# keonlee9420/Comprehensive-Transformer-TTS

Measured on AMD Instinct MI355X. Metric: mel-frames/sec (train step) LJSpeech batch=16, 1/2/4/8 MI355X, higher is better.
Workload: dtype f32; 1 GPU; LJSpeech transformer_fs2 batch=16/GPU seq<=128->mel<=1024x80; full train step fwd+loss+bwd+clip+Adam, dropout on; workload_detail=supervised durations (BASELINE configs[1]), global_batch=16, valid_frames_per_gpu=11992, padded_frames_per_gpu=16384, launch_mode=hipgraph(fwd+bwd | clip+adam), parallelism=dp1

## Files before the change

comprehensive-transformer-tts_amd/_lib.py:

```python
import ctypes as C
import os

_HERE = os.path.dirname(os.path.abspath(__file__))
LIB_PATH = os.environ.get("CTTS_LIB") or os.path.join(_HERE, "csrc", "libctts_hip.so")

_c_f32p = C.c_void_p
_i32, _i64, _f32, _u32, _vp = C.c_int32, C.c_int64, C.c_float, C.c_uint32, C.c_void_p


class GemmDesc(C.Structure):
    _fields_ = [
        ("A", _vp), ("B", _vp), ("C", _vp),
        ("M", _i32), ("N", _i32), ("K", _i32),
        ("lda", _i64), ("ldb", _i64), ("ldc", _i64),
        ("a_kc", _i32), ("b_kc", _i32),
        ("nb0", _i32), ("nb1", _i32),
        ("sA0", _i64), ("sA1", _i64), ("sB0", _i64), ("sB1", _i64), ("sC0", _i64), ("sC1", _i64),
        ("lens", _vp),
        ("lim_m", _i32), ("lim_n", _i32), ("lim_k", _i32),
        ("conv_T", _i32), ("conv_pad", _i32), ("conv_cin", _i32), ("conv_on_b", _i32),
        ("split_k", _i32),
        ("alpha", _f32),
        ("bias", _vp),
        ("Z", _vp), ("ldz", _i64),
# ... 83 lines not shown
    "ctts_gemm_takes_weight_stationary": [C.POINTER(GemmDesc)],
    "ctts_gemm_takes_bf16_split": [C.POINTER(GemmDesc)],
    "ctts_gemm_takes_planes": [C.POINTER(GemmDesc)],
    "ctts_split_planes": [C.POINTER(SplitTask), C.c_int, _vp],
    "ctts_rowdot_heads": [_vp, _vp, _vp, C.c_int, C.c_int, C.c_int, C.c_int, _vp],
    "ctts_mel_prepare": [_vp, C.c_int, C.c_int, _vp, _vp],
    "ctts_mel_spectrogram": [_vp, _vp, _vp, _vp, _vp, _vp, _vp, _i64, C.c_int, C.c_int, C.c_int, C.c_int, C.c_int, _f32, C.c_int, _vp, _vp],
    "ctts_mha_fwd": [_vp, _vp, _vp, _vp, C.c_int, C.c_int, C.c_int, C.c_int, _f32, _vp],
    "ctts_mha_bwd": [_vp, _vp, _vp, _vp, _vp, _vp, _vp, _vp, _vp, C.c_int, C.c_int, C.c_int, C.c_int, _f32, C.c_int, _vp, _vp],
    "ctts_relmha_fwd": [_vp, _vp, _vp, _vp, _vp, _vp, C.c_int, C.c_int, C.c_int, C.c_int, _f32, _f32, _vp, _u32, _vp],
    "ctts_relmha_bwd": [_vp, _vp, _vp, _vp, _vp, _vp, _vp, _vp, _vp, _vp, _vp, _vp, _vp, C.c_int, C.c_int, C.c_int, C.c_int,
                        _f32, _f32, _vp, _u32, _vp],
    "ctts_weighted_colsum": [_vp, _vp, _vp, _i64, C.c_int, _f32, C.c_int, _vp, _vp, _vp],
    "ctts_epilogue_bwd": [_vp, _vp, _vp, _vp, _vp, _vp, _i64, C.c_int, C.c_int, _f32, _vp, _u32, _f32, C.c_int, _vp, _vp, _vp],
    "ctts_row_tile_map": [_vp, C.c_int, C.c_int, C.c_int, _vp, _vp],
    "ctts_batch_tile_map": [_vp] + [C.c_int] * 9 + [_vp, C.c_size_t, _vp],
    "ctts_conv_weight_repack": [_vp, _vp, C.c_int, C.c_int, C.c_int, C.c_int, _vp],
    "ctts_lr_index": [_vp, C.c_int, C.c_int, _vp, C.c_int, C.c_int, C.c_int, _vp, _vp, _vp, _vp],
    "ctts_lr_gather_fwd": [_vp, _vp, _vp, C.c_int, C.c_int, C.c_int, C.c_int, _vp],
    "ctts_lr_gather_bwd": [_vp, _vp, _vp, C.c_int, C.c_int, C.c_int, C.c_int, _vp],
    "ctts_embedding_fwd": [_vp, _vp, _vp, _i64, C.c_int, C.c_int, _vp],
    "ctts_embedding_bwd": [_vp, _vp, _vp, _i64, C.c_int, C.c_int, C.c_int, C.c_int, _vp, _vp],
    "ctts_positions": [_vp, C.c_int, _i64, C.c_int, C.c_int, _vp, _vp],
    "ctts_cwt_pitch": [_vp, _i64, C.c_int, _vp, _vp, _f32, _vp, C.c_int, _f32, _f32, _f32, C.c_int, _vp, _vp, _vp, C.c_int, C.c_int, C.c_int, _vp],
    "ctts_layernorm_fwd": [_vp, _vp, _vp, _vp, _vp, _vp, C.c_int, C.c_int, _f32, _f32, _vp, _u32, _vp, _vp, _vp],
    "ctts_layernorm_bwd": [_vp, _vp, _vp, _vp, _vp, _vp, _vp, _vp, C.c_int, C.c_int, _f32, _vp, _u32, _vp, C.c_int, _vp, _vp, _vp, _vp],
    "ctts_colstats": [_vp, _vp, C.c_int, C.c_int, _vp, _vp],
    "ctts_bn_finalize": [_vp, C.c_int, C.c_int, _f32, _f32, _vp, _vp, _vp, _vp, _vp, _vp],
    "ctts_bn_apply": [_vp, _vp, _vp, _vp, _vp, _vp, C.c_int, C.c_int, C.c_int, _f32, _vp, _u32, _vp, _vp],
    "ctts_bn_bwd_reduce": [_vp, _vp, _vp, _vp, _vp, _vp, _vp, C.c_int, C.c_int, C.c_int, _f32, _vp, _u32, _vp, _vp],
    "ctts_bn_bwd_apply": [_vp, _vp, _vp, _vp, _vp, _vp, _vp, _vp, _vp, _vp, C.c_int, C.c_int, C.c_int, _f32, _vp,
# ... 140 lines not shown
    lib.ctts_pitch_track_workspace_bytes.restype = C.c_size_t
    lib.ctts_pitch_track_workspace_bytes.argtypes = []
    lib.ctts_trim_silence_workspace_bytes.restype = C.c_size_t
    lib.ctts_trim_silence_workspace_bytes.argtypes = [C.c_int, C.c_int, C.c_int]
    lib.ctts_dtw_workspace_bytes.restype = C.c_size_t
    lib.ctts_dtw_workspace_bytes.argtypes = [C.c_int, C.c_int, C.c_int]
    lib.ctts_loudness_workspace_bytes.restype = C.c_size_t
    lib.ctts_loudness_workspace_bytes.argtypes = [C.c_int, C.c_int]
    lib.ctts_stoi_workspace_bytes.restype = C.c_size_t
    lib.ctts_stoi_workspace_bytes.argtypes = [C.c_int, C.c_int]
    lib.ctts_si_sdr_workspace_bytes.restype = C.c_size_t
    lib.ctts_si_sdr_workspace_bytes.argtypes = [C.c_int, C.c_int]
    lib.ctts_mr_stft_workspace_bytes.restype = C.c_size_t
    lib.ctts_mr_stft_workspace_bytes.argtypes = [C.c_int, C.c_int, C.c_int, C.c_int]
    lib.ctts_batch_tile_map_ints.restype = C.c_size_t
    lib.ctts_batch_tile_map_ints.argtypes = [C.c_int, C.c_int, C.c_int, C.c_int]
    lib.ctts_relmha_workspace_floats.restype = C.c_size_t
    lib.ctts_relmha_workspace_floats.argtypes = [C.c_int, C.c_int, C.c_int]
    _lib = lib
    return lib


def check(status, what):
    if status != 0:
        msg = load().ctts_last_error().decode(errors="replace")
        raise CttsError(f"{what} failed with status {status}: {msg}")
```

comprehensive-transformer-tts_amd/csrc/batch_plan.h:

```cpp
#pragma once
#include <stdint.h>
#ifdef __HIPCC__
#define BP_HD __host__ __device__ __forceinline__
#else
#define BP_HD inline
#endif

struct BatchPlanGeom {
  int M, N, K;
  int BM, BN, BK;
  int nbatch, nb1;
  int lim_m, lim_n, lim_k;
  int write_all;
  int nbins;
};

constexpr int BATCH_PLAN_HDR = 4;

BP_HD int batch_plan_tiles_m(const BatchPlanGeom& g) { return (g.M + g.BM - 1) / g.BM; }
BP_HD int batch_plan_tiles_n(const BatchPlanGeom& g) { return (g.N + g.BN - 1) / g.BN; }
BP_HD long batch_plan_items(const BatchPlanGeom& g) { return (long)g.nbatch * batch_plan_tiles_m(g) * batch_plan_tiles_n(g); }

BP_HD bool batch_plan_fits(const BatchPlanGeom& g) {
  const long tiles = (long)batch_plan_tiles_m(g) * batch_plan_tiles_n(g);
// ... 36 lines not shown
  for (int y = 0; y < g.nbatch; ++y) {
    const BatchPlanBatch o = batch_plan_batch(g, lens[y / g.nb1]);
    const int a = o.act_m * o.act_n;
    total += a;
    if (o.work > me.work || (o.work == me.work && y < z)) act_before += a;
    if (y < z) rest_before += tiles - a;
  }
  n_active = total;
  const int tm = tile / tiles_n, tn = tile - tm * tiles_n;
  const int act_in = (tm < me.act_m ? tm : me.act_m) * me.act_n + (tm < me.act_m ? (tn < me.act_n ? tn : me.act_n) : 0);
  if (tm < me.act_m && tn < me.act_n) return batch_plan_snake(act_before + act_in, total, g.nbins);
  return total + rest_before + (tile - act_in);
}

BP_HD int batch_plan_listed(const BatchPlanGeom& g, int n_active) { return g.write_all ? (int)batch_plan_items(g) : n_active; }
```

comprehensive-transformer-tts_amd/csrc/gemm.hip:

```cpp
#include "ctts_common.h"
#include "gemm_common.h"
#include "batch_plan.h"
#include <stdlib.h>
#include <type_traits>

namespace {

#ifndef CTTS_BK
#define CTTS_BK 32
#endif
#ifndef CTTS_GEMM_WAVES
#define CTTS_GEMM_WAVES 2
#endif
constexpr int BK = CTTS_BK;
constexpr int KC_LD = BK + 4;
constexpr int KCH = BK / 4;
static_assert(BK == 32 || BK == 64, "BK must be 32 or 64");


__device__ __forceinline__ bool rows_in_padding(const int32_t* row_lens, int row_T, int row_halo, int first, int last) {
  const int b0 = first / row_T;
  return b0 == last / row_T && (first - b0 * row_T) >= row_lens[b0] + row_halo;
}

// ... 379 lines not shown
__device__ __forceinline__ void fetch_frag(const float* s, int ext0, int l31, int h, int ksub, float (&f)[16]) {
  if (KC) {
    const float4* p = reinterpret_cast<const float4*>(s + (ext0 + l31) * LD + ksub + h * 16);
#pragma unroll
    for (int q = 0; q < 4; ++q) {
      float4 v = p[q];
      f[4 * q + 0] = v.x; f[4 * q + 1] = v.y; f[4 * q + 2] = v.z; f[4 * q + 3] = v.w;
    }
  } else {
    const float* p = s + (ksub + h * 16) * LD + ext0 + l31;
#pragma unroll
    for (int j = 0; j < 16; ++j) f[j] = p[j * LD];
  }
}

template <int BM, int BN, bool A_KC, bool B_KC, bool CONV, Fetch FETCH>
__global__ __launch_bounds__(256, CTTS_GEMM_WAVES) void gemm_tile_kernel(const ctts_gemm_desc d) {
  using FT = FetchTraits<FETCH>;
  constexpr int WAVES_N = BN >= 64 ? 2 : 1, WAVES_M = 4 / WAVES_N;
  constexpr int WM = BM / WAVES_M, WN = BN / WAVES_N, MT = WM / 32, NT = WN / 32;
  constexpr int A_LD = A_KC ? KC_LD : BM + 4;
  constexpr int B_LD = B_KC ? KC_LD : BN + 4;
  constexpr int A_SZ = A_KC ? BM * KC_LD : BK * (BM + 4);
  constexpr int B_SZ = B_KC ? BN * KC_LD : BK * (BN + 4);
  __shared__ __attribute__((aligned(16))) float smem[A_SZ + B_SZ];
  float* sA = smem;
  float* sB = smem + A_SZ;
  int z = blockIdx.z;
  const int split = blockIdx.y;
  const bool limited = FT::kLensLimits && (FT::kLensGiven || d.lens);
  const int tiles_n = (d.N + BN - 1) / BN;
  int wg, tm;
  bool scheduled_active = false;
  if constexpr (FT::kNaturalOrder) {
    wg = blockIdx.x;
    if (d.tile_map && !natural_order(d)) {
      const int32_t* plan = d.tile_map;
      const unsigned lin = blockIdx.z * gridDim.x + blockIdx.x;
      if (plan[2] == (int32_t)(gridDim.x * gridDim.z) && plan[3] == batch_plan_key(batch_plan_geom(d, BM, BN, 1))) {
        if (lin >= (unsigned)plan[1]) return;
        batch_plan_unpack(plan[BATCH_PLAN_HDR + lin], z, wg);
        if (z >= (int)gridDim.z || wg >= (int)gridDim.x) return;
      }
    }
    tm = wg / tiles_n;
// ... 2 lines not shown
    int r = wg / tiles_n;
    if (d.tile_group_n > 0) {
      const int g = d.tile_group_n, ngroups = tiles_n / g, mways = 8 / ngroups;
      const int x = blockIdx.x & 7, i = blockIdx.x >> 3;
      r = (i / g) * mways + x / ngroups;
      wg = r * tiles_n + (x % ngroups) * g + i % g;
    }
    tm = d.tile_map[1 + r];
    scheduled_active = FT::kTrustSchedule && r < d.tile_map[0];
  } else if (FT::kTileOrders && natural_order(d)) {
    wg = blockIdx.x;
    tm = wg / tiles_n;
  } else {
    xcd_tile_order(gridDim.x, tiles_n, true, wg, tm);
  }
  const int z0 = z / d.nb1, z1 = z - z0 * d.nb1;
  int Mv, Nv, Kv;
  batch_limits(d, z0, limited, Mv, Nv, Kv);
  const int row0 = tm * BM, col0 = (wg % tiles_n) * BN;
  float* Cb = d.C + z0 * d.sC0 + z1 * d.sC1;
  const bool zero_outside = limited && d.split_overwrite && d.split_k <= 1;
  if (row0 >= Mv || col0 >= Nv) {
    if (zero_outside && row0 < d.M && col0 < d.N) zero_outside_limits(d, Cb, row0, col0, BM, BN, Mv, Nv, true);
    return;
  }
  if (zero_outside && (row0 + BM > Mv || col0 + BN > Nv)) zero_outside_limits(d, Cb, row0, col0, BM, BN, Mv, Nv, false);
  float* Cs = Cb;
  if (d.split_k > 1) Cs += (long)split * d.M * d.ldc;
  if (A_KC && d.row_lens && !scheduled_active &&
      padded_tile_zeroed(d, FT::kPadFillOwnSplit ? Cs : Cb, row0, col0, BM, min(BN, Nv - col0), Mv)) return;
  int k_begin, k_end;
  if (!split_k_range(d, Kv, BK, split, k_begin, k_end)) return;

  ConvView cv{d.conv_T, d.conv_pad, d.conv_cin};
  ConvView nocv{1, 0, 1};
  constexpr bool CONV_A = CONV && A_KC;
  constexpr bool CONV_B = CONV && !A_KC && !B_KC;
  using LA = Loader<FETCH, A_KC, BM, CONV_A>;
  using LB = Loader<FETCH, B_KC, BN, CONV_B>;
  LA la; LB lb;
  la.init(d.A + z0 * d.sA0 + z1 * d.sA1, d.lda, row0, Mv, CONV_A ? cv : nocv, threadIdx.x);
  lb.init(d.B + z0 * d.sB0 + z1 * d.sB1, d.ldb, col0, Nv, CONV_B ? cv : nocv, threadIdx.x);

  const int lane = threadIdx.x & 63, wave = threadIdx.x >> 6;
  const int l31 = lane & 31, h = lane >> 5;
  const int wm0 = (wave / WAVES_N) * WM, wn0 = (wave % WAVES_N) * WN;
  floatx16 acc[MT][NT];
#pragma unroll
  for (int i = 0; i < MT; ++i)
#pragma unroll
    for (int j = 0; j < NT; ++j)
#pragma unroll
      for (int r = 0; r < 16; ++r) acc[i][j][r] = 0.f;

  constexpr bool KSKIP = !A_KC && !B_KC;
  auto kblock_active = [&](int k0) -> bool {
    if (!KSKIP || !d.row_lens) return true;
    return !rows_in_padding(d.row_lens, d.row_T, d.row_halo, k0, min(k0 + BK, k_end) - 1);
  };
  float4 ra[LA::NV], rb[LB::NV];
  bool act_cur = kblock_active(k_begin);
  if (act_cur) {
    la.load(k_begin, k_end, ra);
    lb.load(k_begin, k_end, rb);
    la.store(sA, ra);
    lb.store(sB, rb);
  }
  __syncthreads();
  for (int k0 = k_begin; k0 < k_end; k0 += BK) {
    const bool has_next = (k0 + BK) < k_end;
    const bool act_next = has_next && kblock_active(k0 + BK);
    if (act_next) {
      la.load(k0 + BK, k_end, ra);
      lb.load(k0 + BK, k_end, rb);
    }
    if (act_cur) {
#pragma unroll
      for (int ksub = 0; ksub < BK; ksub += 32) {
        float fa[MT][16], fb[NT][16];
#pragma unroll
        for (int i = 0; i < MT; ++i) fetch_frag<A_KC, A_LD>(sA, wm0 + i * 32, l31, h, ksub, fa[i]);
#pragma unroll
        for (int j = 0; j < NT; ++j) fetch_frag<B_KC, B_LD>(sB, wn0 + j * 32, l31, h, ksub, fb[j]);
#ifdef CTTS_GEMM_SETPRIO
        __builtin_amdgcn_s_setprio(CTTS_GEMM_SETPRIO);
#endif
#pragma unroll
        for (int kk = 0; kk < 16; ++kk)
#pragma unroll
          for (int i = 0; i < MT; ++i)
#pragma unroll
            for (int j = 0; j < NT; ++j)
              acc[i][j] = __builtin_amdgcn_mfma_f32_32x32x2f32(fa[i][kk], fb[j][kk], acc[i][j], 0, 0, 0);
#ifdef CTTS_GEMM_SETPRIO
        __builtin_amdgcn_s_setprio(0);
#endif
      }
    }
    if (KSKIP && !act_cur && !act_next) continue;
    __syncthreads();
    if (act_next) {
      la.store(sA, ra);
      lb.store(sB, rb);
    }
    __syncthreads();
    act_cur = act_next;
  }
  gemm_epilogue_auto<MT, NT>(d, acc, Cs, z, row0, col0, wm0, wn0, l31, h, Mv, Nv);
}

constexpr int X6_PROW = 64, X6_PLANE = 128 * X6_PROW;
__device__ __forceinline__ int x6_chunk(int row, int c) { return c ^ ((row >> 2) & 3); }
typedef __bf16 x6_bf16x8 __attribute__((ext_vector_type(8)));

typedef __bf16 x6_bf16x2 __attribute__((ext_vector_type(2)));
typedef float x6_floatx2 __attribute__((ext_vector_type(2)));
__device__ __forceinline__ unsigned x6_round_pair(float& a, float& b) {
  const x6_floatx2 v = {a, b};
  const unsigned p = __builtin_bit_cast(unsigned, __builtin_convertvector(v, x6_bf16x2));
  a -= __uint_as_float(p << 16);
  b -= __uint_as_float(p & 0xFFFF0000u);
  return p;
}
// ... 370 lines not shown
    const unsigned long long m = __ballot(a);
    if (a) map[1 + n_act + __popcll(m & ((1ULL << lane) - 1ULL))] = tm;
    n_act += __popcll(m);
  }
  int n_in = 0;
  for (int base = 0; base < tiles; base += 64) {
    const int tm = base + lane;
    const bool a = tm < tiles && inactive(tm);
    const unsigned long long m = __ballot(a);
    if (a) map[1 + n_act + n_in + __popcll(m & ((1ULL << lane) - 1ULL))] = tm;
    n_in += __popcll(m);
  }
  if (lane == 0) map[0] = n_act;
}

__global__ __launch_bounds__(256) void batch_tile_map_kernel(const BatchPlanGeom g, const int32_t* __restrict__ lens, int32_t* __restrict__ map) {
  const int n_items = (int)batch_plan_items(g), tiles = n_items / g.nbatch;
  for (int i = blockIdx.x * 256 + threadIdx.x; i < n_items; i += gridDim.x * 256) {
    const int z = i / tiles, tile = i - z * tiles;
    int n_active;
    const int slot = batch_plan_slot(g, lens, z, tile, n_active);
    map[BATCH_PLAN_HDR + slot] = batch_plan_pack(z, tile);
    if (i == 0) {
      map[0] = n_active;
      map[1] = batch_plan_listed(g, n_active);
      map[2] = n_items;
      map[3] = batch_plan_key(g);
    }
  }
}

__global__ __launch_bounds__(256) void splitk_reduce_kernel(const ctts_gemm_desc d, int BM, int kround) {
  const int z = blockIdx.z, z0 = z / d.nb1, z1 = z - z0 * d.nb1;
  int Mv, Nv, Kv;
  batch_limits(d, z0, true, Mv, Nv, Kv);
  const bool ow = d.split_overwrite != 0;
  const int nact = Kv > 0 ? gemm_split_range(Kv, d.split_k, kround, 0).nonempty : 0;
  if (nact == 0 && !ow) return;
  const long ldp = gemm_partial_ld(d.N);
  const int n4 = (int)(ldp >> 2);
// ... 49 lines not shown
}

static BatchPlanGeom batch_map_geom(int nb0, int nb1, int M, int N, int K, int lim_m, int lim_n, int lim_k, int write_all) {
  static int cus = 0;
  if (!cus) {
    int dev = 0;
    hipDeviceProp_t prop;
    cus = (hipGetDevice(&dev) == hipSuccess && hipGetDeviceProperties(&prop, dev) == hipSuccess && prop.multiProcessorCount > 0)
              ? prop.multiProcessorCount : 256;
    cus = ctts_env_int("CTTS_BATCH_BINS", cus);
    if (cus < 1) cus = 256;
  }
  return BatchPlanGeom{M, N, K, 64, 64, BK, nb0 * nb1, nb1, lim_m != 0, lim_n != 0, lim_k != 0, write_all != 0, cus};
}

extern "C" size_t ctts_batch_tile_map_ints(int nb0, int nb1, int M, int N) {
  if (nb0 < 1 || nb1 < 1 || M < 1 || N < 1 || (long)nb0 * nb1 > 32767) return 0;
  const BatchPlanGeom g = batch_map_geom(nb0, nb1, M, N, 1, 0, 0, 0, 0);
  return batch_plan_fits(g) ? (size_t)(BATCH_PLAN_HDR + batch_plan_items(g)) : 0;
}

extern "C" int ctts_batch_tile_map(const int32_t* lens, int nb0, int nb1, int M, int N, int K, int lim_m, int lim_n, int lim_k,
                                   int write_all, int32_t* tile_map, size_t map_ints, void* stream) {
  CTTS_REQUIRE(lens && tile_map && K >= 0, "ctts_batch_tile_map: bad arguments");
  const size_t need = ctts_batch_tile_map_ints(nb0, nb1, M, N);
  CTTS_REQUIRE(need > 0, "ctts_batch_tile_map: %d x %d batches of [%d, %d] do not fit a plan (ctts_batch_tile_map_ints)", nb0, nb1, M, N);
  CTTS_REQUIRE(map_ints >= need, "ctts_batch_tile_map: tile_map holds %zu int32, %zu needed", map_ints, need);
  const BatchPlanGeom g = batch_map_geom(nb0, nb1, M, N, K, lim_m, lim_n, lim_k, write_all);
  const long blocks = (batch_plan_items(g) + 255) / 256;
  hipLaunchKernelGGL(batch_tile_map_kernel, dim3((unsigned)(blocks < 64 ? blocks : 64)), dim3(256), 0, (hipStream_t)stream, g, lens, tile_map);
  CTTS_CHECK_LAUNCH("ctts_batch_tile_map");
  return 0;
}

static bool x6_plan(const ctts_gemm_desc& d) {
  const int on = d.bf16_split;
  static const long min_tiles = ctts_env_int("CTTS_X6_MIN_TILES", 384);
  if (on < 1 || !d.a_kc || !d.b_kc || d.nb0 * d.nb1 != 1 || d.split_k > 1 || d.E || d.lens || d.conv_on_b) return false;
  if (d.K < 256 || d.K % BK || d.N % 128 || d.M < 1024) return false;
  if (d.conv_T > 0 && d.conv_cin % 4) return false;
  if (on != 2 && on != 4 && (long)((d.M + 127) / 128) * (d.N / 128) < min_tiles) return false;
  return vec_ok(d) && buf_ok(d);
}

static bool x6tn_plan(const ctts_gemm_desc& d) {
// ... 164 lines not shown
    case CTTS_GEMM_SCALAR64: rc = for_layout<true>(t, [&](auto a, auto b, auto c) { return launch_tile<64, 64, a(), b(), c(), Fetch::Scalar>(t, st); }); break;
#ifndef CTTS_NO_BUF
    case CTTS_GEMM_BUF128: rc = for_layout<true>(t, [&](auto a, auto b, auto c) { return launch_tile<128, 128, a(), b(), c(), Fetch::Buffer>(t, st); }); break;
    case CTTS_GEMM_BUF_K2: rc = for_layout<true>(t, [&](auto a, auto b, auto c) { return launch_buf_k2<a(), b(), c()>(t, st); }); break;
    case CTTS_GEMM_BUF_NARROW: rc = for_layout<false>(t, [&](auto a, auto b, auto c) { return launch_tile<128, 32, a(), b(), c(), Fetch::Buffer>(t, st); }); break;
    case CTTS_GEMM_BUF64: rc = for_layout<true>(t, [&](auto a, auto b, auto c) { return launch_tile<64, 64, a(), b(), c(), Fetch::Buffer>(t, st); }); break;
#endif
    case CTTS_GEMM_VEC128: rc = for_layout<true>(t, [&](auto a, auto b, auto c) { return launch_tile<128, 128, a(), b(), c(), Fetch::Vec>(t, st); }); break;
    case CTTS_GEMM_X6TN: rc = x6tn_launch(t, st); break;
    default: rc = for_layout<true>(t, [&](auto a, auto b, auto c) { return launch_tile<64, 64, a(), b(), c(), Fetch::Vec>(t, st); }); break;
  }
  if (rc != 0 || !split || d.split_out) return rc;
  return splitk_reduce(d_user, r.info.tile_m, r.info.k_granule, st);
}

extern "C" int ctts_gemm_route(const ctts_gemm_desc* dp, ctts_gemm_route_info* info) {
  CTTS_REQUIRE(info != nullptr, "ctts_gemm_route: null info");
  *info = ctts_gemm_route_info{CTTS_GEMM_NONE, 0, 0, 0, 0};
  ctts_gemm_desc d;
  GemmRoute r;
  const int rc = gemm_plan(dp, d, r);
  if (rc == 0) *info = r.info;
  return rc < 0 ? rc : 0;
}

static int route_kind(const ctts_gemm_desc* dp) {
  if (!dp) return CTTS_GEMM_NONE;
  const ctts_gemm_desc d = gemm_normalized(*dp);
  GemmRoute r;
  gemm_route(d, r);
// ... 25 lines not shown
```

comprehensive-transformer-tts_amd/kernels.py:

```python
import collections
import ctypes as C

import torch

from . import _lib
from ._lib import GemmDesc

ACT_NONE, ACT_RELU, ACT_GELU, ACT_TANH, ACT_SWISH = 0, 1, 2, 3, 4


def _stream():
    return C.c_void_p(torch.cuda.current_stream().cuda_stream)


def _p(t, offset=0):
    if t is None:
        return None
    if not t.is_cuda:
        raise _lib.CttsError("ctts kernels need device (HIP) tensors; got a CPU tensor - no CPU fallback exists")
    return t.data_ptr() + offset * t.element_size()


def _f32c(t, name):
    if t.dtype != torch.float32 or not t.is_contiguous():
# ... 391 lines not shown
def gemm_takes_weight_stationary(A, B, Cout, M, N, K, lda, ldb, ldc, a_kc=True, b_kc=True, **kw):
    return _gemm_takes("weight_stationary", (A, B, Cout, M, N, K, lda, ldb, ldc, a_kc, b_kc), kw)


def gemm_ws_enable(on):
    return bool(_lib.load().ctts_gemm_ws_enable(1 if on else 0))


def row_tile_map(row_lens, row_T, row_halo, M):
    tm = torch.empty(1 + (M + 63) // 64, dtype=torch.int32, device=row_lens.device)
    lib = _lib.load()
    _lib.check(lib.ctts_row_tile_map(_p(row_lens), int(row_T), int(row_halo), int(M), _p(tm), _stream()), "ctts_row_tile_map")
    return tm


def batch_tile_map(lens, nb1, M, N, K, lim, write_all):
    lib = _lib.load()
    n = lib.ctts_batch_tile_map_ints(int(lens.numel()), int(nb1), int(M), int(N))
    if n == 0:
        return None
    tm = torch.empty(n, dtype=torch.int32, device=lens.device)
    _lib.check(lib.ctts_batch_tile_map(_p(lens), int(lens.numel()), int(nb1), int(M), int(N), int(K), int(lim[0]), int(lim[1]), int(lim[2]),
                                       int(bool(write_all)), _p(tm), n, _stream()), "ctts_batch_tile_map")
    return tm


def conv_dgrad_weights(weights):
    if not weights:
        return []
    outs = [torch.empty(cin, k * cout, dtype=torch.float32, device=w.device) for w, cout, cin, k in weights]
    arr = (_lib.RepackTask * len(weights))()
    for t, (w, cout, cin, k), o in zip(arr, weights, outs):
        t.src, t.dst, t.cout, t.cin, t.k = _p(_f32c(w, "conv weight (GEMM-major)")), _p(o), int(cout), int(cin), int(k)
    _lib.check(_lib.load().ctts_conv_dgrad_weights(arr, len(arr), _stream()), "ctts_conv_dgrad_weights")
    return outs


def conv_weight_repack(src, dst, cout, cin, k, mode):
    lib = _lib.load()
# ... 1481 lines not shown
```

comprehensive-transformer-tts_amd/ops.py:

```python
import contextlib
import math
import os as _os

import torch

from . import kernels as K
from .kernels import ACT_NONE, ACT_RELU, ACT_GELU, ACT_TANH, ACT_SWISH


_FUSE_GRAD_ACCUM = False


def set_grad_accumulation_fusion(flag):
    global _FUSE_GRAD_ACCUM
    _FUSE_GRAD_ACCUM = bool(flag)


def grad_accumulation_fusion():
    return _FUSE_GRAD_ACCUM


def _grad_of(p):
    if not _FUSE_GRAD_ACCUM or p is None or not p.requires_grad:
        return None
# ... 448 lines not shown
        _PLANES[kind][w.data_ptr()] = (pl, _wstamp(w))


def clear_dgrad_weights():
    _DGRAD_W.clear()
    _PLANES["fwd"].clear()
    _PLANES["dgrad"].clear()


class PadRows:

    def __init__(self, lens, T):
        self.lens, self.T = lens, int(T)
        self._maps = {}
        self._batch_maps = {}

    def tile_map(self, halo, M):
        key = (int(halo), int(M))
        if key not in self._maps:
            self._maps[key] = K.row_tile_map(self.lens, self.T, halo, M)
        return self._maps[key]


    def batch_map(self, A, B, Cout, lim, write_all):
        key = (tuple(Cout.shape), int(A.shape[-1]), tuple(lim), bool(write_all))
        if key not in self._batch_maps:
            plan = None
            nb1, (M, N), Kd = (Cout.shape[1] if Cout.dim() == 4 else 1), Cout.shape[-2:], A.shape[-1]
            if Cout.is_cuda and Cout.dim() >= 3 and Cout.shape[0] * nb1 * -(-M // 64) * -(-N // 64) > _BATCH_ORDER_MIN_ITEMS:
                args, views = K.gemm_views(A, B, Cout, lens=self.lens)
                route = K.gemm_route(*args, **views, lens=self.lens, lim=lim, split_overwrite=write_all)
                if route.kind == "buf64":
                    plan = K.batch_tile_map(self.lens, nb1, M, N, Kd, lim, write_all)
            self._batch_maps[key] = plan
        return self._batch_maps[key]


def _pad_rows(pad_rows):
    if pad_rows is None or isinstance(pad_rows, PadRows):
        return pad_rows
    return PadRows(pad_rows[0], pad_rows[1])


def linear(x, w, b=None, act=ACT_NONE, alpha=1.0, residual=None, rowscale=None, p_drop=0.0, drop=None, pad_rows=None, link=None,
           link_role=0):
    p_drop, seed, off = _drop_args(p_drop, drop)
    return _LinearConv.apply(x, w, b, residual, rowscale, act, alpha, p_drop, seed, off, 0, 0, _pad_rows(pad_rows), link, link_role)


def conv1d(x, w, b=None, act=ACT_NONE, alpha=1.0, residual=None, rowscale=None, p_drop=0.0, drop=None, pad_rows=None, link=None,
# ... 109 lines not shown


def layer_norm_res(x, gamma, beta, eps, planes_for=None):
    want = planes_for is not None and consumer_takes_planes(x, *planes_for)
    return _LayerNormRes.apply(x, gamma, beta, eps, want)


def layer_norm(x, gamma, beta, eps, rowscale=None, p_drop=0.0, drop=None):
    p_drop, seed, off = _drop_args(p_drop, drop)
    return _LayerNorm.apply(x, gamma, beta, eps, rowscale, p_drop, seed, off)


_ATTN_SPLIT_K = int(_os.environ.get("CTTS_ATTN_SPLIT_K", "1"))
_BATCH_ORDER = _os.environ.get("CTTS_BATCH_ORDER", "balanced")
_BATCH_ORDER_MIN_ITEMS = 256


def _attn_split_k(nbatch, T, dh):
    tiles = -(-T // 64) * -(-dh // 64) * nbatch
    return _ATTN_SPLIT_K if (_ATTN_SPLIT_K > 1 and tiles < 1536 and T >= 512) else 1


_FUSED_ATTN = {"1": True, "0": False}.get(_os.environ.get("CTTS_FUSED_ATTN", "auto"), None)
_ATTN_Q_SPLIT = int(_os.environ.get("CTTS_ATTN_Q_SPLIT", "0"))


def set_fused_attention(flag):
    global _FUSED_ATTN
    _FUSED_ATTN = flag if flag is None else bool(flag)

# ... 49 lines not shown
        ctx.n_heads = n_heads
        ctx.pad_rows = pr
        return out

    @staticmethod
    def backward(ctx, dO):
        qkv, P, lens, O = ctx.saved_tensors
        H, pr, bg = ctx.n_heads, ctx.pad_rows, _SelfAttention._bgemm
        dO = dO.contiguous()
        B, T, C3 = qkv.shape
        dh = C3 // 3 // H
        scale = dh ** -0.5
        sk = _attn_split_k(B * H, T, dh)
        dqkv = torch.empty_like(qkv)
        (q, k, v), (dq, dk, dv), (dOh,) = _heads(qkv, H, 3), _heads(dqkv, H, 3), _heads(dO, H)
        bg(pr, P.transpose(-1, -2), dOh, dv, lens, (1, 0, 1), split_k=sk, split_overwrite=True)
        Dv = K.rowdot_heads(dO, O, H)
        dP = torch.empty_like(P)
        bg(pr, dOh, v.transpose(-1, -2), dP, lens, (1, 1, 0), E=P, rowsub=Dv)
        bg(pr, dP, k, dq, lens, (1, 0, 1), alpha=scale, split_k=sk, split_overwrite=True)
        bg(pr, dP.transpose(-1, -2), q, dk, lens, (1, 0, 1), alpha=scale, split_k=sk, split_overwrite=True)
        return dqkv, None, None, None


def self_attention(qkv, lens_i32, n_heads, pad_rows=None):
    want = _FUSED_ATTN if _FUSED_ATTN is not None else not (torch.is_grad_enabled() and qkv.requires_grad)
    if want and K.mha_supported(qkv.shape[-1] // 3, n_heads):
        return _FusedSelfAttention.apply(qkv, lens_i32, n_heads)
    return _SelfAttention.apply(qkv, lens_i32, n_heads, pad_rows)


class _LRGather(torch.autograd.Function):
    @staticmethod
    def forward(ctx, x, mel2ph, cum):
# ... 829 lines not shown
```

include/ctts.h:

```cpp
#ifndef CTTS_H
#define CTTS_H
#include <stddef.h>
#include <stdint.h>

#ifdef __cplusplus
extern "C" {
#endif

const char* ctts_last_error(void);
int ctts_version(void);

typedef struct ctts_gemm_desc {
  const float* A; const float* B; float* C;
  int32_t M, N, K;
  int64_t lda, ldb, ldc;
  int32_t a_kc, b_kc;
  int32_t nb0, nb1;
  int64_t sA0, sA1, sB0, sB1, sC0, sC1;
  const int32_t* lens;
  int32_t lim_m, lim_n, lim_k;
  int32_t conv_T, conv_pad, conv_cin, conv_on_b;
  int32_t split_k;
  float alpha;
  const float* bias;
// ... 49 lines not shown
int ctts_gemm_takes_planes(const ctts_gemm_desc* d);
typedef struct ctts_split_task { const float* src; uint16_t* dst; int64_t rows, cols, ld; } ctts_split_task;
int ctts_split_planes(const ctts_split_task* tasks, int ntasks, void* stream);

int ctts_rowdot_heads(const float* a, const float* b, float* out, int B, int T, int H, int dh, void* stream);

int ctts_weighted_colsum(const float* x, const float* w, float* out, int64_t rows, int C, float scale, int accumulate, void* ws, float* parts,
                         void* stream);

int ctts_epilogue_bwd(const float* dy, const float* rowscale, const float* z, float* dz, float* gm, float* dbias, int64_t rows, int C,
                      int act, float p_drop, const uint64_t* seed, uint32_t drop_offset, float bias_scale, int accumulate_bias,
                      void* ws, float* parts, void* stream);

int ctts_row_tile_map(const int32_t* row_lens, int row_T, int row_halo, int M, int32_t* tile_map, void* stream);

size_t ctts_batch_tile_map_ints(int nb0, int nb1, int M, int N);
int ctts_batch_tile_map(const int32_t* lens, int nb0, int nb1, int M, int N, int K, int lim_m, int lim_n, int lim_k, int write_all,
                        int32_t* tile_map, size_t map_ints, void* stream);

int ctts_conv_weight_repack(const float* src, float* dst, int cout, int cin, int k, int mode, void* stream);

int ctts_lr_index(const void* dur, int dur_is_float, int round_mode, const uint8_t* pad, int B, int Ts, int Tm,
                  int32_t* mel2ph, int64_t* mel_len, int32_t* cum, void* stream);
int ctts_lr_gather_fwd(const float* x, const int32_t* mel2ph, float* out, int B, int Ts, int Tm, int C, void* stream);
int ctts_lr_gather_bwd(const float* dy, const int32_t* cum, float* dx, int B, int Ts, int Tm, int C, void* stream);

int ctts_cwt_pitch(const float* spec, int64_t ld_spec, int nscale, const float* f0_mean, const float* f0_std, float std_scale,
                   const float* uv, int uv_chan, float eps, float mel_min, float mel_max, int f0_bin, float* f0, float* f0_denorm,
                   int64_t* ids, int B, int T, int width, void* stream);

int ctts_positions(const void* src, int src_is_float, int64_t stride, int B, int T, int32_t* pos, void* stream);

int ctts_layernorm_fwd(const float* x, const float* gamma, const float* beta, float* y, float* mean, float* rstd,
// ... 247 lines not shown
```

Baseline: 672,200 mel-frames/s.

## Group attention-backward dV, dQ, dK batched GEMMs into one length-balanced launch

Adds a grouped GEMM kernel that runs up to three same-shape, length-limited batched GEMMs in one launch, using a combined tile plan that orders active tiles by work across all groups. Attention backward uses it for dV, dQ and dK, deferring dV until after dP is computed, when split-K is off. The aim is to cut launch count and fill the GPU better with small per-head attention GEMMs. In exchange the kernel is launched with bounds of 8 waves per SIMD and carries larger shared memory covering both layouts, and the tile-map API gains a groups argument.

```diff
diff --git a/comprehensive-transformer-tts_amd/_lib.py b/comprehensive-transformer-tts_amd/_lib.py
--- a/comprehensive-transformer-tts_amd/_lib.py
+++ b/comprehensive-transformer-tts_amd/_lib.py
@@ -121,7 +121,8 @@
     "ctts_weighted_colsum": [_vp, _vp, _vp, _i64, C.c_int, _f32, C.c_int, _vp, _vp, _vp],
     "ctts_epilogue_bwd": [_vp, _vp, _vp, _vp, _vp, _vp, _i64, C.c_int, C.c_int, _f32, _vp, _u32, _f32, C.c_int, _vp, _vp, _vp],
     "ctts_row_tile_map": [_vp, C.c_int, C.c_int, C.c_int, _vp, _vp],
-    "ctts_batch_tile_map": [_vp] + [C.c_int] * 9 + [_vp, C.c_size_t, _vp],
+    "ctts_batch_tile_map": [_vp] + [C.c_int] * 10 + [_vp, C.c_size_t, _vp],
+    "ctts_gemm_grouped": [_vp, C.c_int, _vp, _vp],
     "ctts_conv_weight_repack": [_vp, _vp, C.c_int, C.c_int, C.c_int, C.c_int, _vp],
     "ctts_lr_index": [_vp, C.c_int, C.c_int, _vp, C.c_int, C.c_int, C.c_int, _vp, _vp, _vp, _vp],
     "ctts_lr_gather_fwd": [_vp, _vp, _vp, C.c_int, C.c_int, C.c_int, C.c_int, _vp],
@@ -292,7 +293,7 @@
     lib.ctts_mr_stft_workspace_bytes.restype = C.c_size_t
     lib.ctts_mr_stft_workspace_bytes.argtypes = [C.c_int, C.c_int, C.c_int, C.c_int]
     lib.ctts_batch_tile_map_ints.restype = C.c_size_t
-    lib.ctts_batch_tile_map_ints.argtypes = [C.c_int, C.c_int, C.c_int, C.c_int]
+    lib.ctts_batch_tile_map_ints.argtypes = [C.c_int, C.c_int, C.c_int, C.c_int, C.c_int]
     lib.ctts_relmha_workspace_floats.restype = C.c_size_t
     lib.ctts_relmha_workspace_floats.argtypes = [C.c_int, C.c_int, C.c_int]
     _lib = lib
diff --git a/comprehensive-transformer-tts_amd/csrc/batch_plan.h b/comprehensive-transformer-tts_amd/csrc/batch_plan.h
--- a/comprehensive-transformer-tts_amd/csrc/batch_plan.h
+++ b/comprehensive-transformer-tts_amd/csrc/batch_plan.h
@@ -74,3 +74,38 @@
 }
 
 BP_HD int batch_plan_listed(const BatchPlanGeom& g, int n_active) { return g.write_all ? (int)batch_plan_items(g) : n_active; }
+
+constexpr int BATCH_PLAN_MAX_GROUPS = 3;
+
+BP_HD bool batch_plan_group_fits(const BatchPlanGeom& g, int groups) {
+  return groups >= 1 && groups <= BATCH_PLAN_MAX_GROUPS && batch_plan_fits(g) && g.nbatch <= 16383 &&
+         batch_plan_items(g) * groups <= (1L << 24);
+}
+BP_HD int32_t batch_plan_group_pack(int grp, int z, int tile) { return (int32_t)(((uint32_t)grp << 30) | ((uint32_t)z << 16) | (uint32_t)tile); }
+BP_HD void batch_plan_group_unpack(int32_t e, int& grp, int& z, int& tile) {
+  grp = (int)((uint32_t)e >> 30); z = (int)(((uint32_t)e >> 16) & 0x3FFF); tile = e & 0xFFFF;
+}
+
+BP_HD int batch_plan_group_slot(const BatchPlanGeom& g, int groups, const int32_t* lens, int grp, int z, int tile, int& n_active) {
+  const int tiles_n = batch_plan_tiles_n(g), tiles = batch_plan_tiles_m(g) * tiles_n;
+  const BatchPlanBatch me = batch_plan_batch(g, lens[z / g.nb1]);
+  int heavier = 0, equal = 0, equal_before = 0, rest_before = 0, total = 0;
+  for (int y = 0; y < g.nbatch; ++y) {
+    const BatchPlanBatch o = batch_plan_batch(g, lens[y / g.nb1]);
+    const int a = o.act_m * o.act_n;
+    total += a;
+    if (o.work > me.work) heavier += a;
+    else if (o.work == me.work) { equal += a; if (y < z) equal_before += a; }
+    if (y < z) rest_before += tiles - a;
+  }
+  n_active = groups * total;
+  const int tm = tile / tiles_n, tn = tile - tm * tiles_n;
+  const int act_in = (tm < me.act_m ? tm : me.act_m) * me.act_n + (tm < me.act_m ? (tn < me.act_n ? tn : me.act_n) : 0);
+  if (tm < me.act_m && tn < me.act_n)
+    return batch_plan_snake(groups * heavier + grp * equal + equal_before + act_in, n_active, g.nbins);
+  return n_active + grp * (g.nbatch * tiles - total) + rest_before + (tile - act_in);
+}
+
+BP_HD int batch_plan_group_listed(const BatchPlanGeom& g, int groups, int n_active) {
+  return g.write_all ? groups * (int)batch_plan_items(g) : n_active;
+}
diff --git a/comprehensive-transformer-tts_amd/csrc/gemm.hip b/comprehensive-transformer-tts_amd/csrc/gemm.hip
--- a/comprehensive-transformer-tts_amd/csrc/gemm.hip
+++ b/comprehensive-transformer-tts_amd/csrc/gemm.hip
@@ -417,21 +417,123 @@
   }
 }
 
+template <int BM, int BN, bool A_KC, bool B_KC>
+constexpr int tile_smem_floats() { return (A_KC ? BM * KC_LD : BK * (BM + 4)) + (B_KC ? BN * KC_LD : BK * (BN + 4)); }
+
 template <int BM, int BN, bool A_KC, bool B_KC, bool CONV, Fetch FETCH>
-__global__ __launch_bounds__(256, CTTS_GEMM_WAVES) void gemm_tile_kernel(const ctts_gemm_desc d) {
+__device__ __forceinline__ void gemm_tile_body(const ctts_gemm_desc& d, float* smem, const int z, const int split, const int wg, const int tm,
+                                               const bool scheduled_active) {
   using FT = FetchTraits<FETCH>;
   constexpr int WAVES_N = BN >= 64 ? 2 : 1, WAVES_M = 4 / WAVES_N;
   constexpr int WM = BM / WAVES_M, WN = BN / WAVES_N, MT = WM / 32, NT = WN / 32;
   constexpr int A_LD = A_KC ? KC_LD : BM + 4;
   constexpr int B_LD = B_KC ? KC_LD : BN + 4;
   constexpr int A_SZ = A_KC ? BM * KC_LD : BK * (BM + 4);
-  constexpr int B_SZ = B_KC ? BN * KC_LD : BK * (BN + 4);
-  __shared__ __attribute__((aligned(16))) float smem[A_SZ + B_SZ];
   float* sA = smem;
   float* sB = smem + A_SZ;
+  const bool limited = FT::kLensLimits && (FT::kLensGiven || d.lens);
+  const int tiles_n = (d.N + BN - 1) / BN;
+  const int z0 = z / d.nb1, z1 = z - z0 * d.nb1;
+  int Mv, Nv, Kv;
+  batch_limits(d, z0, limited, Mv, Nv, Kv);
+  const int row0 = tm * BM, col0 = (wg % tiles_n) * BN;
+  float* Cb = d.C + z0 * d.sC0 + z1 * d.sC1;
+  const bool zero_outside = limited && d.split_overwrite && d.split_k <= 1;
+  if (row0 >= Mv || col0 >= Nv) {
+    if (zero_outside && row0 < d.M && col0 < d.N) zero_outside_limits(d, Cb, row0, col0, BM, BN, Mv, Nv, true);
+    return;
+  }
+  if (zero_outside && (row0 + BM > Mv || col0 + BN > Nv)) zero_outside_limits(d, Cb, row0, col0, BM, BN, Mv, Nv, false);
+  float* Cs = Cb;
+  if (d.split_k > 1) Cs += (long)split * d.M * d.ldc;
+  if (A_KC && d.row_lens && !scheduled_active &&
+      padded_tile_zeroed(d, FT::kPadFillOwnSplit ? Cs : Cb, row0, col0, BM, min(BN, Nv - col0), Mv)) return;
+  int k_begin, k_end;
+  if (!split_k_range(d, Kv, BK, split, k_begin, k_end)) return;
+
+  ConvView cv{d.conv_T, d.conv_pad, d.conv_cin};
+  ConvView nocv{1, 0, 1};
+  constexpr bool CONV_A = CONV && A_KC;
+  constexpr bool CONV_B = CONV && !A_KC && !B_KC;
+  using LA = Loader<FETCH, A_KC, BM, CONV_A>;
+  using LB = Loader<FETCH, B_KC, BN, CONV_B>;
+  LA la; LB lb;
+  la.init(d.A + z0 * d.sA0 + z1 * d.sA1, d.lda, row0, Mv, CONV_A ? cv : nocv, threadIdx.x);
+  lb.init(d.B + z0 * d.sB0 + z1 * d.sB1, d.ldb, col0, Nv, CONV_B ? cv : nocv, threadIdx.x);
+
+  const int lane = threadIdx.x & 63, wave = threadIdx.x >> 6;
+  const int l31 = lane & 31, h = lane >> 5;
+  const int wm0 = (wave / WAVES_N) * WM, wn0 = (wave % WAVES_N) * WN;
+  floatx16 acc[MT][NT];
+#pragma unroll
+  for (int i = 0; i < MT; ++i)
+#pragma unroll
+    for (int j = 0; j < NT; ++j)
+#pragma unroll
+      for (int r = 0; r < 16; ++r) acc[i][j][r] = 0.f;
+
+  constexpr bool KSKIP = !A_KC && !B_KC;
+  auto kblock_active = [&](int k0) -> bool {
+    if (!KSKIP || !d.row_lens) return true;
+    return !rows_in_padding(d.row_lens, d.row_T, d.row_halo, k0, min(k0 + BK, k_end) - 1);
+  };
+  float4 ra[LA::NV], rb[LB::NV];
+  bool act_cur = kblock_active(k_begin);
+  if (act_cur) {
+    la.load(k_begin, k_end, ra);
+    lb.load(k_begin, k_end, rb);
+    la.store(sA, ra);
+    lb.store(sB, rb);
+  }
+  __syncthreads();
+  for (int k0 = k_begin; k0 < k_end; k0 += BK) {
+    const bool has_next = (k0 + BK) < k_end;
+    const bool act_next = has_next && kblock_active(k0 + BK);
+    if (act_next) {
+      la.load(k0 + BK, k_end, ra);
+      lb.load(k0 + BK, k_end, rb);
+    }
+    if (act_cur) {
+#pragma unroll
+      for (int ksub = 0; ksub < BK; ksub += 32) {
+        float fa[MT][16], fb[NT][16];
+#pragma unroll
+        for (int i = 0; i < MT; ++i) fetch_frag<A_KC, A_LD>(sA, wm0 + i * 32, l31, h, ksub, fa[i]);
+#pragma unroll
+        for (int j = 0; j < NT; ++j) fetch_frag<B_KC, B_LD>(sB, wn0 + j * 32, l31, h, ksub, fb[j]);
+#ifdef CTTS_GEMM_SETPRIO
+        __builtin_amdgcn_s_setprio(CTTS_GEMM_SETPRIO);
+#endif
+#pragma unroll
+        for (int kk = 0; kk < 16; ++kk)
+#pragma unroll
+          for (int i = 0; i < MT; ++i)
+#pragma unroll
+            for (int j = 0; j < NT; ++j)
+              acc[i][j] = __builtin_amdgcn_mfma_f32_32x32x2f32(fa[i][kk], fb[j][kk], acc[i][j], 0, 0, 0);
+#ifdef CTTS_GEMM_SETPRIO
+        __builtin_amdgcn_s_setprio(0);
+#endif
+      }
+    }
+    if (KSKIP && !act_cur && !act_next) continue;
+    __syncthreads();
+    if (act_next) {
+      la.store(sA, ra);
+      lb.store(sB, rb);
+    }
+    __syncthreads();
+    act_cur = act_next;
+  }
+  gemm_epilogue_auto<MT, NT>(d, acc, Cs, z, row0, col0, wm0, wn0, l31, h, Mv, Nv);
+}
+
+template <int BM, int BN, bool A_KC, bool B_KC, bool CONV, Fetch FETCH>
+__global__ __launch_bounds__(256, CTTS_GEMM_WAVES) void gemm_tile_kernel(const ctts_gemm_desc d) {
+  using FT = FetchTraits<FETCH>;
+  __shared__ __attribute__((aligned(16))) float smem[tile_smem_floats<BM, BN, A_KC, B_KC>()];
   int z = blockIdx.z;
   const int split = blockIdx.y;
-  const bool limited = FT::kLensLimits && (FT::kLensGiven || d.lens);
   const int tiles_n = (d.N + BN - 1) / BN;
   int wg, tm;
   bool scheduled_active = false;
@@ -464,99 +566,36 @@
   } else {
     xcd_tile_order(gridDim.x, tiles_n, true, wg, tm);
   }
-  const int z0 = z / d.nb1, z1 = z - z0 * d.nb1;
-  int Mv, Nv, Kv;
-  batch_limits(d, z0, limited, Mv, Nv, Kv);
-  const int row0 = tm * BM, col0 = (wg % tiles_n) * BN;
-  float* Cb = d.C + z0 * d.sC0 + z1 * d.sC1;
-  const bool zero_outside = limited && d.split_overwrite && d.split_k <= 1;
-  if (row0 >= Mv || col0 >= Nv) {
-    if (zero_outside && row0 < d.M && col0 < d.N) zero_outside_limits(d, Cb, row0, col0, BM, BN, Mv, Nv, true);
-    return;
-  }
-  if (zero_outside && (row0 + BM > Mv || col0 + BN > Nv)) zero_outside_limits(d, Cb, row0, col0, BM, BN, Mv, Nv, false);
-  float* Cs = Cb;
-  if (d.split_k > 1) Cs += (long)split * d.M * d.ldc;
-  if (A_KC && d.row_lens && !scheduled_active &&
-      padded_tile_zeroed(d, FT::kPadFillOwnSplit ? Cs : Cb, row0, col0, BM, min(BN, Nv - col0), Mv)) return;
-  int k_begin, k_end;
-  if (!split_k_range(d, Kv, BK, split, k_begin, k_end)) return;
-
-  ConvView cv{d.conv_T, d.conv_pad, d.conv_cin};
-  ConvView nocv{1, 0, 1};
-  constexpr bool CONV_A = CONV && A_KC;
-  constexpr bool CONV_B = CONV && !A_KC && !B_KC;
-  using LA = Loader<FETCH, A_KC, BM, CONV_A>;
-  using LB = Loader<FETCH, B_KC, BN, CONV_B>;
-  LA la; LB lb;
-  la.init(d.A + z0 * d.sA0 + z1 * d.sA1, d.lda, row0, Mv, CONV_A ? cv : nocv, threadIdx.x);
-  lb.init(d.B + z0 * d.sB0 + z1 * d.sB1, d.ldb, col0, Nv, CONV_B ? cv : nocv, threadIdx.x);
-
-  const int lane = threadIdx.x & 63, wave = threadIdx.x >> 6;
-  const int l31 = lane & 31, h = lane >> 5;
-  const int wm0 = (wave / WAVES_N) * WM, wn0 = (wave % WAVES_N) * WN;
-  floatx16 acc[MT][NT];
-#pragma unroll
-  for (int i = 0; i < MT; ++i)
-#pragma unroll
-    for (int j = 0; j < NT; ++j)
-#pragma unroll
-      for (int r = 0; r < 16; ++r) acc[i][j][r] = 0.f;
-
-  constexpr bool KSKIP = !A_KC && !B_KC;
-  auto kblock_active = [&](int k0) -> bool {
-    if (!KSKIP || !d.row_lens) return true;
-    return !rows_in_padding(d.row_lens, d.row_T, d.row_halo, k0, min(k0 + BK, k_end) - 1);
-  };
-  float4 ra[LA::NV], rb[LB::NV];
-  bool act_cur = kblock_active(k_begin);
-  if (act_cur) {
-    la.load(k_begin, k_end, ra);
-    lb.load(k_begin, k_end, rb);
-    la.store(sA, ra);
-    lb.store(sB, rb);
-  }
-  __syncthreads();
-  for (int k0 = k_begin; k0 < k_end; k0 += BK) {
-    const bool has_next = (k0 + BK) < k_end;
-    const bool act_next = has_next && kblock_active(k0 + BK);
-    if (act_next) {
-      la.load(k0 + BK, k_end, ra);
-      lb.load(k0 + BK, k_end, rb);
-    }
-    if (act_cur) {
-#pragma unroll
-      for (int ksub = 0; ksub < BK; ksub += 32) {
-        float fa[MT][16], fb[NT][16];
-#pragma unroll
-        for (int i = 0; i < MT; ++i) fetch_frag<A_KC, A_LD>(sA, wm0 + i * 32, l31, h, ksub, fa[i]);
-#pragma unroll
-        for (int j = 0; j < NT; ++j) fetch_frag<B_KC, B_LD>(sB, wn0 + j * 32, l31, h, ksub, fb[j]);
-#ifdef CTTS_GEMM_SETPRIO
-        __builtin_amdgcn_s_setprio(CTTS_GEMM_SETPRIO);
-#endif
-#pragma unroll
-        for (int kk = 0; kk < 16; ++kk)
-#pragma unroll
-          for (int i = 0; i < MT; ++i)
-#pragma unroll
-            for (int j = 0; j < NT; ++j)
-              acc[i][j] = __builtin_amdgcn_mfma_f32_32x32x2f32(fa[i][kk], fb[j][kk], acc[i][j], 0, 0, 0);
-#ifdef CTTS_GEMM_SETPRIO
-        __builtin_amdgcn_s_setprio(0);
-#endif
-      }
-    }
-    if (KSKIP && !act_cur && !act_next) continue;
-    __syncthreads();
-    if (act_next) {
-      la.store(sA, ra);
-      lb.store(sB, rb);
-    }
-    __syncthreads();
-    act_cur = act_next;
-  }
-  gemm_epilogue_auto<MT, NT>(d, acc, Cs, z, row0, col0, wm0, wn0, l31, h, Mv, Nv);
+  gemm_tile_body<BM, BN, A_KC, B_KC, CONV, FETCH>(d, smem, z, split, wg, tm, scheduled_active);
+}
+
+struct GemmGroupArgs {
+  ctts_gemm_desc d[BATCH_PLAN_MAX_GROUPS];
+  const int32_t* plan;
+  int groups;
+};
+
+template <int BM, int BN, Fetch FETCH>
+__global__ __launch_bounds__(256, 8) void gemm_tile_group_kernel(const GemmGroupArgs a) {
+  constexpr int SM_NN = tile_smem_floats<BM, BN, true, false>(), SM_TN = tile_smem_floats<BM, BN, false, false>();
+  __shared__ __attribute__((aligned(16))) float smem[SM_NN > SM_TN ? SM_NN : SM_TN];
+  const ctts_gemm_desc& d0 = a.d[0];
+  const int tiles_n = (d0.N + BN - 1) / BN, tiles = ((d0.M + BM - 1) / BM) * tiles_n, nbatch = d0.nb0 * d0.nb1;
+  const unsigned lin = blockIdx.x, per_group = (unsigned)tiles * nbatch;
+  int grp = (int)(lin / per_group), z = (int)((lin - grp * per_group) / tiles), wg = (int)(lin - grp * per_group - (unsigned)z * tiles);
+  if (a.plan) {
+    const int32_t* plan = a.plan;
+    if (plan[2] == (int32_t)gridDim.x && plan[3] == batch_plan_key(batch_plan_geom(d0, BM, BN, 1))) {
+      if (lin >= (unsigned)plan[1]) return;
+      batch_plan_group_unpack(plan[BATCH_PLAN_HDR + lin], grp, z, wg);
+      if (z >= nbatch || wg >= tiles) return;
+    }
+  }
+  if (grp >= a.groups) return;
+  grp = __builtin_amdgcn_readfirstlane(grp); z = __builtin_amdgcn_readfirstlane(z); wg = __builtin_amdgcn_readfirstlane(wg);
+  const ctts_gemm_desc& d = a.d[grp];
+  if (d.a_kc) gemm_tile_body<BM, BN, true, false, false, FETCH>(d, smem, z, 0, wg, wg / tiles_n, false);
+  else gemm_tile_body<BM, BN, false, false, false, FETCH>(d, smem, z, 0, wg, wg / tiles_n, false);
 }
 
 constexpr int X6_PROW = 64, X6_PLANE = 128 * X6_PROW;
@@ -957,16 +996,17 @@
   if (lane == 0) map[0] = n_act;
 }
 
-__global__ __launch_bounds__(256) void batch_tile_map_kernel(const BatchPlanGeom g, const int32_t* __restrict__ lens, int32_t* __restrict__ map) {
-  const int n_items = (int)batch_plan_items(g), tiles = n_items / g.nbatch;
+__global__ __launch_bounds__(256) void batch_tile_map_kernel(const BatchPlanGeom g, const int groups, const int32_t* __restrict__ lens,
+                                                             int32_t* __restrict__ map) {
+  const int per_group = (int)batch_plan_items(g), n_items = groups * per_group, tiles = per_group / g.nbatch;
   for (int i = blockIdx.x * 256 + threadIdx.x; i < n_items; i += gridDim.x * 256) {
-    const int z = i / tiles, tile = i - z * tiles;
+    const int grp = i / per_group, z = (i - grp * per_group) / tiles, tile = i - grp * per_group - z * tiles;
     int n_active;
-    const int slot = batch_plan_slot(g, lens, z, tile, n_active);
-    map[BATCH_PLAN_HDR + slot] = batch_plan_pack(z, tile);
+    const int slot = batch_plan_group_slot(g, groups, lens, grp, z, tile, n_active);
+    map[BATCH_PLAN_HDR + slot] = batch_plan_group_pack(grp, z, tile);
     if (i == 0) {
       map[0] = n_active;
-      map[1] = batch_plan_listed(g, n_active);
+      map[1] = batch_plan_group_listed(g, groups, n_active);
       map[2] = n_items;
       map[3] = batch_plan_key(g);
     }
@@ -1046,21 +1086,23 @@
   return BatchPlanGeom{M, N, K, 64, 64, BK, nb0 * nb1, nb1, lim_m != 0, lim_n != 0, lim_k != 0, write_all != 0, cus};
 }
 
-extern "C" size_t ctts_batch_tile_map_ints(int nb0, int nb1, int M, int N) {
+extern "C" size_t ctts_batch_tile_map_ints(int nb0, int nb1, int M, int N, int groups) {
   if (nb0 < 1 || nb1 < 1 || M < 1 || N < 1 || (long)nb0 * nb1 > 32767) return 0;
   const BatchPlanGeom g = batch_map_geom(nb0, nb1, M, N, 1, 0, 0, 0, 0);
-  return batch_plan_fits(g) ? (size_t)(BATCH_PLAN_HDR + batch_plan_items(g)) : 0;
+  if (groups == 1) return batch_plan_fits(g) ? (size_t)(BATCH_PLAN_HDR + batch_plan_items(g)) : 0;
+  return batch_plan_group_fits(g, groups) ? (size_t)(BATCH_PLAN_HDR + groups * batch_plan_items(g)) : 0;
 }
 
 extern "C" int ctts_batch_tile_map(const int32_t* lens, int nb0, int nb1, int M, int N, int K, int lim_m, int lim_n, int lim_k,
-                                   int write_all, int32_t* tile_map, size_t map_ints, void* stream) {
+                                   int write_all, int groups, int32_t* tile_map, size_t map_ints, void* stream) {
   CTTS_REQUIRE(lens && tile_map && K >= 0, "ctts_batch_tile_map: bad arguments");
-  const size_t need = ctts_batch_tile_map_ints(nb0, nb1, M, N);
-  CTTS_REQUIRE(need > 0, "ctts_batch_tile_map: %d x %d batches of [%d, %d] do not fit a plan (ctts_batch_tile_map_ints)", nb0, nb1, M, N);
+  const size_t need = ctts_batch_tile_map_ints(nb0, nb1, M, N, groups);
+  CTTS_REQUIRE(need > 0, "ctts_batch_tile_map: %d group(s) of %d x %d batches of [%d, %d] do not fit a plan (ctts_batch_tile_map_ints)", groups,
+               nb0, nb1, M, N);
   CTTS_REQUIRE(map_ints >= need, "ctts_batch_tile_map: tile_map holds %zu int32, %zu needed", map_ints, need);
   const BatchPlanGeom g = batch_map_geom(nb0, nb1, M, N, K, lim_m, lim_n, lim_k, write_all);
-  const long blocks = (batch_plan_items(g) + 255) / 256;
-  hipLaunchKernelGGL(batch_tile_map_kernel, dim3((unsigned)(blocks < 64 ? blocks : 64)), dim3(256), 0, (hipStream_t)stream, g, lens, tile_map);
+  const long blocks = (groups * batch_plan_items(g) + 255) / 256;
+  hipLaunchKernelGGL(batch_tile_map_kernel, dim3((unsigned)(blocks < 64 ? blocks : 64)), dim3(256), 0, (hipStream_t)stream, g, groups, lens, tile_map);
   CTTS_CHECK_LAUNCH("ctts_batch_tile_map");
   return 0;
 }
@@ -1255,6 +1297,44 @@
   return splitk_reduce(d_user, r.info.tile_m, r.info.k_granule, st);
 }
 
+extern "C" int ctts_gemm_grouped(const ctts_gemm_desc* descs, int count, const int32_t* plan, void* stream) {
+#ifdef CTTS_NO_BUF
+  ctts_set_error("ctts_gemm_grouped: built without the buffer kernels");
+  return -1;
+#else
+  CTTS_REQUIRE(descs && count >= 1 && count <= BATCH_PLAN_MAX_GROUPS, "ctts_gemm_grouped: 1 to %d descriptors", BATCH_PLAN_MAX_GROUPS);
+  GemmGroupArgs a{};
+  bool natural = false;
+  for (int i = 0; i < count; ++i) {
+    ctts_gemm_desc in = descs[i];
+    in.tile_map = nullptr;
+    ctts_gemm_desc& d = a.d[i];
+    GemmRoute r;
+    const int rc = gemm_plan(&in, d, r);
+    if (rc < 0) return rc;
+    CTTS_REQUIRE(rc == 0, "ctts_gemm_grouped: member %d has an empty output", i);
+    CTTS_REQUIRE(r.info.kind == CTTS_GEMM_BUF64 && d.split_k <= 1 && !d.row_lens && d.conv_T <= 0 && d.lens && (d.lim_m || d.lim_n || d.lim_k),
+                 "ctts_gemm_grouped: member %d is not a length-limited batched launch of the 64 x 64 buffer kernel without split-K "
+                 "(route kind %d)", i, r.info.kind);
+    CTTS_REQUIRE(!d.b_kc, "ctts_gemm_grouped: member %d has a K-contiguous B operand (NN and TN layouts are instantiated)", i);
+    const ctts_gemm_desc& f = a.d[0];
+    CTTS_REQUIRE(d.M == f.M && d.N == f.N && d.K == f.K && d.nb0 == f.nb0 && d.nb1 == f.nb1 && d.lens == f.lens && !d.lim_m == !f.lim_m &&
+                 !d.lim_n == !f.lim_n && !d.lim_k == !f.lim_k && !d.split_overwrite == !f.split_overwrite,
+                 "ctts_gemm_grouped: member %d differs from member 0 in extents, batches, lens, limits or split_overwrite", i);
+    natural = natural || r.natural_order;
+  }
+  const BatchPlanGeom g = batch_plan_geom(a.d[0], 64, 64, 1);
+  CTTS_REQUIRE(batch_plan_group_fits(g, count), "ctts_gemm_grouped: %d groups of %d batches of [%d, %d] do not fit one launch", count, g.nbatch,
+               g.M, g.N);
+  a.plan = natural ? nullptr : plan;
+  a.groups = count;
+  hipLaunchKernelGGL((gemm_tile_group_kernel<64, 64, Fetch::BufferPartial>), dim3((unsigned)(count * batch_plan_items(g))), dim3(256), 0,
+                     reinterpret_cast<hipStream_t>(stream), a);
+  CTTS_CHECK_LAUNCH("ctts_gemm_grouped");
+  return 0;
+#endif
+}
+
 extern "C" int ctts_gemm_route(const ctts_gemm_desc* dp, ctts_gemm_route_info* info) {
   CTTS_REQUIRE(info != nullptr, "ctts_gemm_route: null info");
   *info = ctts_gemm_route_info{CTTS_GEMM_NONE, 0, 0, 0, 0};
diff --git a/comprehensive-transformer-tts_amd/kernels.py b/comprehensive-transformer-tts_amd/kernels.py
--- a/comprehensive-transformer-tts_amd/kernels.py
+++ b/comprehensive-transformer-tts_amd/kernels.py
@@ -429,15 +429,24 @@
     return tm
 
 
-def batch_tile_map(lens, nb1, M, N, K, lim, write_all):
-    lib = _lib.load()
-    n = lib.ctts_batch_tile_map_ints(int(lens.numel()), int(nb1), int(M), int(N))
+def batch_tile_map(lens, nb1, M, N, K, lim, write_all, groups=1):
+    lib = _lib.load()
+    n = lib.ctts_batch_tile_map_ints(int(lens.numel()), int(nb1), int(M), int(N), int(groups))
     if n == 0:
         return None
     tm = torch.empty(n, dtype=torch.int32, device=lens.device)
     _lib.check(lib.ctts_batch_tile_map(_p(lens), int(lens.numel()), int(nb1), int(M), int(N), int(K), int(lim[0]), int(lim[1]), int(lim[2]),
-                                       int(bool(write_all)), _p(tm), n, _stream()), "ctts_batch_tile_map")
+                                       int(bool(write_all)), int(groups), _p(tm), n, _stream()), "ctts_batch_tile_map")
     return tm
+
+
+def bgemm_group(members, plan=None, **kw):
+    descs = (_lib.GemmDesc * len(members))()
+    for i, (A, B, Cout, own) in enumerate(members):
+        args, views = gemm_views(A, B, Cout, own.get("E"), kw.get("lens"))
+        descs[i] = _gemm_desc(*args, **views, **kw, **own)
+    _lib.check(_lib.load().ctts_gemm_grouped(descs, len(members), _p(plan), _stream()), "ctts_gemm_grouped")
+    return [m[2] for m in members]
 
 
 def conv_dgrad_weights(weights):
diff --git a/comprehensive-transformer-tts_amd/ops.py b/comprehensive-transformer-tts_amd/ops.py
--- a/comprehensive-transformer-tts_amd/ops.py
+++ b/comprehensive-transformer-tts_amd/ops.py
@@ -486,6 +486,7 @@
         self.lens, self.T = lens, int(T)
         self._maps = {}
         self._batch_maps = {}
+        self._group_maps = {}
 
     def tile_map(self, halo, M):
         key = (int(halo), int(M))
@@ -506,6 +507,16 @@
                     plan = K.batch_tile_map(self.lens, nb1, M, N, Kd, lim, write_all)
             self._batch_maps[key] = plan
         return self._batch_maps[key]
+
+    def group_map(self, A, B, Cout, lim, write_all, groups):
+        key = (tuple(Cout.shape), int(A.shape[-1]), tuple(lim), bool(write_all), int(groups))
+        if key not in self._group_maps:
+            plan = None
+            if self.batch_map(A, B, Cout, lim, write_all) is not None:
+                nb1, (M, N) = (Cout.shape[1] if Cout.dim() == 4 else 1), Cout.shape[-2:]
+                plan = K.batch_tile_map(self.lens, nb1, M, N, A.shape[-1], lim, write_all, groups)
+            self._group_maps[key] = plan
+        return self._group_maps[key]
 
 
 def _pad_rows(pad_rows):
@@ -645,6 +656,12 @@
 _ATTN_SPLIT_K = int(_os.environ.get("CTTS_ATTN_SPLIT_K", "1"))
 _BATCH_ORDER = _os.environ.get("CTTS_BATCH_ORDER", "balanced")
 _BATCH_ORDER_MIN_ITEMS = 256
+_ATTN_GROUP = _os.environ.get("CTTS_ATTN_GROUP", "1") != "0"
+
+
+def set_attention_group(flag):
+    global _ATTN_GROUP
+    _ATTN_GROUP = bool(flag)
 
 
 def _attn_split_k(nbatch, T, dh):
@@ -724,10 +741,17 @@
         sk = _attn_split_k(B * H, T, dh)
         dqkv = torch.empty_like(qkv)
         (q, k, v), (dq, dk, dv), (dOh,) = _heads(qkv, H, 3), _heads(dqkv, H, 3), _heads(dO, H)
-        bg(pr, P.transpose(-1, -2), dOh, dv, lens, (1, 0, 1), split_k=sk, split_overwrite=True)
+        Pt = P.transpose(-1, -2)
+        group = pr.group_map(Pt, dOh, dv, (1, 0, 1), True, 3) if (_ATTN_GROUP and pr is not None and sk <= 1) else None
+        if group is None:
+            bg(pr, Pt, dOh, dv, lens, (1, 0, 1), split_k=sk, split_overwrite=True)
         Dv = K.rowdot_heads(dO, O, H)
         dP = torch.empty_like(P)
         bg(pr, dOh, v.transpose(-1, -2), dP, lens, (1, 1, 0), E=P, rowsub=Dv)
+        if group is not None:
+            K.bgemm_group([(Pt, dOh, dv, {}), (dP, k, dq, dict(alpha=scale)), (dP.transpose(-1, -2), q, dk, dict(alpha=scale))], group,
+                          lens=lens, lim=(1, 0, 1), split_overwrite=True)
+            return dqkv, None, None, None
         bg(pr, dP, k, dq, lens, (1, 0, 1), alpha=scale, split_k=sk, split_overwrite=True)
         bg(pr, dP.transpose(-1, -2), q, dk, lens, (1, 0, 1), alpha=scale, split_k=sk, split_overwrite=True)
         return dqkv, None, None, None
diff --git a/include/ctts.h b/include/ctts.h
--- a/include/ctts.h
+++ b/include/ctts.h
@@ -87,9 +87,11 @@
 
 int ctts_row_tile_map(const int32_t* row_lens, int row_T, int row_halo, int M, int32_t* tile_map, void* stream);
 
-size_t ctts_batch_tile_map_ints(int nb0, int nb1, int M, int N);
+size_t ctts_batch_tile_map_ints(int nb0, int nb1, int M, int N, int groups);
 int ctts_batch_tile_map(const int32_t* lens, int nb0, int nb1, int M, int N, int K, int lim_m, int lim_n, int lim_k, int write_all,
-                        int32_t* tile_map, size_t map_ints, void* stream);
+                        int groups, int32_t* tile_map, size_t map_ints, void* stream);
+
+int ctts_gemm_grouped(const ctts_gemm_desc* descs, int count, const int32_t* plan, void* stream);
 
 int ctts_conv_weight_repack(const float* src, float* dst, int cout, int cin, int k, int mode, void* stream);
 
```

New measurement: 678,000 mel-frames/s (median of 6 runs). About the same (+0.9%).
